# uibk-uncover/ws-unet

Hardware: AMD Instinct MI355X
Metric: 512x512 grayscale images/sec (UNet predict) (higher is better)
Workload: dtype f16 MFMA on the f16 halves + ONE block-scaled fp4 (e2m1) MFMA per tap pair for both residual cross terms (per-pixel / per-(co, tap) E8M0 scales), fp32 accumulate; planar storage

## Files before the change

ws_unet_amd/csrc/conv3x3_q.hip:

```cpp
#include "wsu_device.h"
#include <cstdlib>

namespace {

constexpr int TW = 32, TH = 16, IW = TW + 2, IH = TH + 2;
constexpr int NPIX = IW * IH;
constexpr int PLANE = NPIX * 16;
constexpr int IN_SEG = (NPIX + 63) / 64;
constexpr int S_LDS = IN_SEG * 256;
constexpr int IN_SLOT = 3 * PLANE + S_LDS;
constexpr int W_GRAN = 9 * 3 * WSU_COB * 16;
constexpr int W_SLOT = W_GRAN + 1024;
constexpr int NIN = 3, NWS = 2;
constexpr int W_BASE = NIN * IN_SLOT;
constexpr int LDS_EXTRA = W_BASE + NWS * W_SLOT;
constexpr int ZERO_BYTES = 3 * IW * 16 + 32;
constexpr int LDS_TOTAL = LDS_EXTRA + 1024 * 4 + 4 * 64 * 4 + 16 + ZERO_BYTES;
static_assert(LDS_TOTAL <= 160 * 1024 && W_SLOT % 1024 == 0, "LDS budget");
constexpr int NLOAD = 4;
constexpr int W_PIECES = W_SLOT / 1024;
constexpr unsigned OOB = 0xFFFFFFF0u;
constexpr int IN_SLOT_H = 2 * PLANE;
constexpr int W_SLOT_H = 9 * 2 * WSU_COB * 16;
template <int FMT> struct QGeo {
// ... 321 lines not shown
    auto q4_reads = [&](auto tp_c, auto ml_c, auto mu_c, u32x4* a4, u32x4* b4, int* sa, int* sb) __attribute__((always_inline)) {
        constexpr int tp = decltype(tp_c)::value, ML = decltype(ml_c)::value, MU = decltype(mu_c)::value;
        constexpr bool single = 2 * tp + 1 >= 9;
        constexpr int t0 = 2 * tp, pix0 = (t0 / 3) * IW + t0 % 3;
        constexpr unsigned wimm = (unsigned)((6 * tp + 2) * 64) * 16u;
        static_assert(!single || (wimm == W4_IMM && (unsigned)pix0 * 16u == B4_IMM), "tap 8");
        const unsigned wbase = single ? x_w4 : x_w, sabase = single ? x_sa4 : x_sa;
        const unsigned bbase = single ? x_b4 : (tp == 1 ? x_b2 : x_b1), sbbase = single ? x_sb0 : (tp == 1 ? x_sb2 : x_sb1);
_Pragma("unroll")
        for (int m = ML; m < MU; ++m) {
            a4[m] = *(lds_cu32x4*)(at(wbase) + wimm + m * 32 * 16);
            sa[m] = *(lds_cuchar*)(at(sabase) + 128 * tp + m * 32);
        }
_Pragma("unroll")
        for (int q = 0; q < RQ; ++q) {
            b4[q] = *(lds_cu32x4*)(at(bbase) + (pix0 + q * IW) * 16);
            sb[q] = *(lds_cint*)(at(sbbase) + (pix0 + q * IW) * 4);
        }
    };
    auto cross_q4 = [&](auto tp_c, auto ms_c, auto first_c) __attribute__((always_inline)) {
        constexpr int ms = decltype(ms_c)::value, ML = ms < 0 ? 0 : ms, MU = ms < 0 ? MH : ms + 1;
        constexpr bool FIRST = decltype(first_c)::value;
        u32x4 a4[2], b4[4]; int sa[2], sb[4];
        q4_reads(tp_c, std::integral_constant<int, ML>{}, std::integral_constant<int, MU>{}, a4, b4, sa, sb);
_Pragma("unroll")
        for (int m = ML; m < MU; ++m)
_Pragma("unroll")
            for (int q = 0; q < RQ; ++q) {
                if constexpr (FIRST) acc[m][q] = wsu_mfma_q4_z(a4[m], b4[q], sa[m], sb[q]);
                else wsu_mfma_q4(a4[m], b4[q], sa[m], sb[q], acc[m][q]);
            }
    };
    constexpr std::false_type not_first{};
    constexpr std::true_type tile_first{};
    auto units_range = [&](auto ms_c, auto lo_c, auto hi_c, auto first_c) __attribute__((always_inline)) {
        constexpr int lo = decltype(lo_c)::value, hi = decltype(hi_c)::value;
        constexpr bool FIRST = decltype(first_c)::value;
        static_assert(!FIRST || lo == 0, "a tile opens with tap pair 0");
        WSU_STATIC_FOR(hi - lo, i, {
            constexpr int tp = lo + i;
            if constexpr (!H) cross_q4(std::integral_constant<int, tp>{}, ms_c, std::integral_constant<bool, FIRST && tp == 0>{});
            main_term(std::integral_constant<int, 2 * tp>{}, ms_c, std::integral_constant<bool, FIRST && H && tp == 0>{});
            if constexpr (2 * tp + 1 < 9) main_term(std::integral_constant<int, 2 * tp + 1>{}, ms_c, not_first);
        });
    };
    constexpr std::integral_constant<int, -1> all_m{};
    struct Frag { u32x4 a[2]; u32x4 b[4]; int sa[2]; int sb[4]; };
    auto load_unit = [&](auto u_c, Frag& f, u32x4* row1) __attribute__((always_inline)) {
        constexpr int u = decltype(u_c)::value, tp = u / 3, k = u % 3;
        if constexpr (k == 0) {
            q4_reads(std::integral_constant<int, tp>{}, std::integral_constant<int, 0>{}, std::integral_constant<int, MH>{}, f.a, f.b, f.sa, f.sb);
        } else {
            constexpr int tap = 2 * tp + k - 1, dy = tap / 3, dx = tap % 3;
_Pragma("unroll")
            for (int m = 0; m < MH; ++m) f.a[m] = *(lds_cu32x4*)(at(a_off) + ((tap * 3) * 64 + m * 32) * 16);
            if constexpr (RQ == 2) {
                if constexpr (dy > 0) f.b[0] = row1[tap - 3];
                else f.b[0] = *(lds_cu32x4*)(at(b_off) + (dy * IW + dx) * 16);
                f.b[1] = row1[tap] = *(lds_cu32x4*)(at(b_off) + ((1 + dy) * IW + dx) * 16);
            } else {
_Pragma("unroll")
                for (int q = 0; q < RQ; ++q) f.b[q] = *(lds_cu32x4*)(at(b_off) + ((q + dy) * IW + dx) * 16);
            }
        }
    };
    auto mma_unit = [&](auto u_c, Frag& f, auto first_c) __attribute__((always_inline)) {
        constexpr int u = decltype(u_c)::value, k = u % 3;
        constexpr bool FIRST = decltype(first_c)::value && u == 0;
        if constexpr (k == 0) {
_Pragma("unroll")
            for (int m = 0; m < MH; ++m)
_Pragma("unroll")
                for (int q = 0; q < RQ; ++q) {
                    if constexpr (FIRST) acc[m][q] = wsu_mfma_q4_z(f.a[m], f.b[q], f.sa[m], f.sb[q]);
                    else wsu_mfma_q4(f.a[m], f.b[q], f.sa[m], f.sb[q], acc[m][q]);
                }
        } else {
_Pragma("unroll")
            for (int m = 0; m < MH; ++m)
_Pragma("unroll")
                for (int q = 0; q < RQ; ++q) wsu_mfma_f16(f.a[m], f.b[q], acc[m][q]);
        }
    };
    auto units_pipelined = [&](auto first_c) __attribute__((always_inline)) {
        constexpr int NU = 14;
        Frag fr[2];
        u32x4 row1[9];
        load_unit(std::integral_constant<int, 0>{}, fr[0], row1);
        WSU_STATIC_FOR(NU, u, {
            if constexpr (u + 1 < NU) load_unit(std::integral_constant<int, u + 1>{}, fr[(u + 1) % 2], row1);
            __builtin_amdgcn_sched_barrier(0);
            mma_unit(u_c, fr[u % 2], first_c);
            __builtin_amdgcn_sched_barrier(0);
        });
    };
    auto units_all = [&](auto ms_c, auto first_c) __attribute__((always_inline)) {
        if constexpr (PIPE && decltype(ms_c)::value < 0) { units_pipelined(first_c); return; }
        units_range(ms_c, std::integral_constant<int, 0>{}, std::integral_constant<int, 5>{}, first_c);
    };

    auto finish_tile = [&]() __attribute__((always_inline)) {
        int l31 = l31_k, hh = hh_k;
        asm volatile("" : "+v"(l31), "+v"(hh));
        const int col = cur.x0 + l31;
        const unsigned hw16 = (unsigned)(a.h * a.w) * 16u;
        const int nco = a.cout >> 4;
        float hz[4][HC > 0 ? HC : 1];
        float vmax = 0.f;
        const float relu_floor = a.relu ? 0.f : -__builtin_inff();
#pragma unroll
        for (int q = 0; q < RQ; ++q)
#pragma unroll
            for (int o = 0; o < (HC > 0 ? HC : 1); ++o) hz[q][o] = 0.f;
        struct QOff { unsigned g0, g1, q, s; };
        auto pair_off = [&](unsigned plane_bytes, unsigned off0, unsigned off1, unsigned soff0, unsigned soff1, bool ok0, bool ok1) __attribute__((always_inline)) {
            const unsigned hp = hh ? plane_bytes : 0u;
            const bool okm = hh ? ok1 : ok0;
            QOff o = {ok0 ? off0 + hp : OOB, ok1 ? off1 + hp : OOB, okm ? (hh ? off1 : off0) + 2u * plane_bytes : OOB, okm ? 3u * plane_bytes + (hh ? soff1 : soff0) : OOB};
            asm volatile("" : "+v"(o.g0), "+v"(o.g1), "+v"(o.q), "+v"(o.s));
            return o;
        };
        constexpr bool YQ = FQ && !H;
        QOff qo[RQ / 2] = {}, qop = {};
        if constexpr (YQ) {
            const unsigned sblk = (unsigned)(((cur.y0 >> 4) * a.tiles_x + (cur.x0 >> 5)) * 512);
_Pragma("unroll")
            for (int rp = 0; rp < RQ / 2; ++rp) {
                const int r0 = RQ * wv + 2 * rp, row0 = cur.y0 + r0;
                qo[rp] = pair_off(hw16, (unsigned)(row0 * a.w + col) * 16u, (unsigned)((row0 + 1) * a.w + col) * 16u,
                                  sblk + (unsigned)(r0 * 32 + l31), sblk + (unsigned)((r0 + 1) * 32 + l31), row0 < a.h && col < a.w, row0 + 1 < a.h && col < a.w);
            }
            if constexpr (POOL) {
                const int hp = a.h >> 1, wp2 = a.w >> 1, ptx = (wp2 + 31) >> 5;
                const int gy0 = (cur.y0 >> 1) + (RQ / 2) * wv, gx = (cur.x0 >> 1) + (l31 >> 1);
                const unsigned php16 = (unsigned)(hp * wp2) * 16u;
                if constexpr (RQ == 4) {
                    const bool okx = !(l31 & 1) && gx < wp2;
                    qop = pair_off(php16, (unsigned)(gy0 * wp2 + gx) * 16u, (unsigned)((gy0 + 1) * wp2 + gx) * 16u,
                                   wsu_q_soff(gy0, gx, ptx), wsu_q_soff(gy0 + 1, gx, ptx), okx && gy0 < hp, okx && gy0 + 1 < hp);
                } else {
                    const unsigned coff = (l31 & 1) ? (unsigned)wsu_q_chunk_bytes(hp, wp2) : 0u;
                    const unsigned off = (unsigned)(gy0 * wp2 + gx) * 16u + coff, soff = wsu_q_soff(gy0, gx, ptx) + coff;
                    const bool ok = gx < wp2 && gy0 < hp;
                    qop = {ok ? off + (hh ? php16 : 0u) : OOB, OOB, (ok && !hh) ? off + 2u * php16 : OOB, (ok && !hh) ? 3u * php16 + soff : OOB};
                    asm volatile("" : "+v"(qop.g0), "+v"(qop.q), "+v"(qop.s));
                }
            }
        }
        auto store_pair_q = [&](const f32x4& X0, const f32x4& Y0, const f32x4& X1, const f32x4& Y1, char* base, unsigned chunk_bytes, const QOff& o, bool have, bool fold) __attribute__((always_inline)) {
            u32x4 g0, g1; uint32_t dh0, dr0, sb0, dh1, dr1, sb1;
            const float mx0 = wsu_q4_pre(X0, Y0, g0, dh0, dr0, sb0);
            const float mx1 = wsu_q4_pre(X1, Y1, g1, dh1, dr1, sb1);
            if (fold) vmax = wsu_max3(vmax, mx0, mx1);
            const u32x4 qg = wsu_q4_pair(dh0, dr0, dh1, dr1);
            const auto rs = __builtin_amdgcn_make_buffer_rsrc(base, 0, have ? (int)chunk_bytes : 0, 0x00020000);
            __builtin_amdgcn_raw_buffer_store_b128(g0, rs, (int)o.g0, 0, 0);
            __builtin_amdgcn_raw_buffer_store_b128(g1, rs, (int)o.g1, 0, 0);
            __builtin_amdgcn_raw_buffer_store_b128(qg, rs, (int)o.q, 0, 0);
            __builtin_amdgcn_raw_buffer_store_b8((unsigned char)(hh ? sb1 : sb0), rs, (int)o.s, 0, 0);
        };
        auto store_one_q = [&](const f32x4& X, const f32x4& Y, char* base, unsigned chunk_bytes, const QOff& o) __attribute__((always_inline)) {
            u32x4 g; uint32_t dh, dr, sb;
            wsu_q4_pre(X, Y, g, dh, dr, sb);
            const u32x4 qg = wsu_q4_single(dh, dr);
            const auto rs = __builtin_amdgcn_make_buffer_rsrc(base, 0, (int)chunk_bytes, 0x00020000);
            __builtin_amdgcn_raw_buffer_store_b128(g, rs, (int)o.g0, 0, 0);
            __builtin_amdgcn_raw_buffer_store_b128(qg, rs, (int)o.q, 0, 0);
            __builtin_amdgcn_raw_buffer_store_b8((unsigned char)sb, rs, (int)o.s, 0, 0);
        };
        auto store_one_h = [&](const f32x4& X, const f32x4& Y, char* base, unsigned plane_bytes, unsigned off, bool ok, bool have) __attribute__((always_inline)) {
            const auto rs = __builtin_amdgcn_make_buffer_rsrc(base, 0, have ? (int)(2u * plane_bytes) : 0, 0x00020000);
            __builtin_amdgcn_raw_buffer_store_b128(wsu_h_granule(X, Y), rs, (int)(ok ? off + (hh ? plane_bytes : 0u) : OOB), 0, 0);
        };
        auto store_one_a = [&](const f32x4& X, const f32x4& Y, char* base, unsigned plane_bytes, unsigned off, bool ok, bool have) __attribute__((always_inline)) {
            uint32_t xh0, xh1, xlo, yh0, yh1, ylo;
            wsu_split4_f16r8(X, WSU_F8_XLO_DIV, xh0, xh1, xlo);
            wsu_split4_f16r8(Y, WSU_F8_XLO_DIV, yh0, yh1, ylo);
            wsu_swap32(xh0, yh0); wsu_swap32(xh1, yh1);
            uint32_t xlp = xlo, ylp = ylo;
            wsu_swap32(xlo, xlp); wsu_swap32(ylo, ylp);
// ... 59 lines not shown
                            const float cx = fmaxf(vx[0][e], vx[1][e]), cy = fmaxf(vy[0][e], vy[1][e]);
                            px[rp][e] = fmaxf(cx, dpp_xor1(cx)); py[rp][e] = fmaxf(cy, dpp_xor1(cy));
                        }
                    }
                });
                if constexpr (POOL) {
                    const int hp = a.h >> 1, wp2 = a.w >> 1;
                    const int gy0 = (cur.y0 >> 1) + (RQ / 2) * wv, gx = (cur.x0 >> 1) + (l31 >> 1);
                    const bool okx = !(l31 & 1) && gx < wp2;
                    const unsigned php16 = (unsigned)(hp * wp2) * 16u;
                    if constexpr (H) {
                        char* base = a.ypool + ((size_t)cur.n * nco + oc) * (2u * php16);
#pragma unroll
                        for (int rp = 0; rp < RQ / 2; ++rp)
                            store_one_h(px[rp], py[rp], base, php16, (unsigned)((gy0 + rp) * wp2 + gx) * 16u, okx && gy0 + rp < hp, true);
                    } else if constexpr (FQ) {
                        const unsigned cbp = (unsigned)wsu_q_chunk_bytes(hp, wp2);
                        char* base = a.ypool + ((size_t)cur.n * nco + oc) * cbp;
                        if constexpr (RQ == 4) {
                            store_pair_q(px[0], py[0], px[1], py[1], base, cbp, qop, true, false);
                        } else if constexpr (cp == 0) {
                            spx = px[0]; spy = py[0];
                        } else {
                            static_assert(cp == 1, "piece 1 closes the pair: its chunk follows piece 0's");
                            const bool odd = (l31 & 1) != 0;
                            f32x4 sx, sy;
_Pragma("unroll")
                            for (int e = 0; e < 4; ++e) { sx[e] = odd ? px[0][e] : spx[e]; sy[e] = odd ? py[0][e] : spy[e]; }
                            store_one_q(sx, sy, base - cbp, 2u * cbp, qop);
                        }
                    } else {
                        char* base = a.ypool + (((size_t)cur.n * nco + oc) * 3) * php16;
#pragma unroll
                        for (int rp = 0; rp < RQ / 2; ++rp)
                            store_one_a(px[rp], py[rp], base, php16, (unsigned)((gy0 + rp) * wp2 + gx) * 16u, okx && gy0 + rp < hp, true);
                    }
                }
            };
            piece(std::integral_constant<int, 0>{});
            piece(std::integral_constant<int, 1>{});
        };
        auto nothing = [](auto) __attribute__((always_inline)) {};
        if constexpr (EPO) {
            constexpr int NHT = 2 * (RQ / 2);
            epi_m(std::integral_constant<int, 0>{}, [&](auto h_c) __attribute__((always_inline)) {
                constexpr int h = decltype(h_c)::value;
                constexpr int lo = 5 * h / NHT, hi = 5 * (h + 1) / NHT;
                if constexpr (hi > lo) units_range(std::integral_constant<int, 1>{}, std::integral_constant<int, lo>{}, std::integral_constant<int, hi>{}, not_first);
            });
            epi_m(std::integral_constant<int, 1>{}, nothing);
        } else {
            WSU_STATIC_FOR(MH, m, { (void)m; epi_m(m_c, nothing); });
        }
        if constexpr (HEAD) {
            const size_t hw = (size_t)a.h * a.w;
#pragma unroll
            for (int q = 0; q < RQ; ++q) {
                const int row = cur.y0 + RQ * wv + q;
#pragma unroll
                for (int o = 0; o < HC; ++o)
                    if (HC == 1 || o < a.head_cout) {
                        uint32_t mine = __builtin_bit_cast(uint32_t, hz[q][o]), other = mine;
                        wsu_swap32(mine, other);
                        const float z = __builtin_bit_cast(float, mine) + __builtin_bit_cast(float, other) + s_hb[o];
                        if (!hh && row < a.h && col < a.w) {
                            const size_t plane = ((size_t)cur.n * a.head_cout + o) * hw;
                            const uint32_t off = (uint32_t)(row * a.w + col);
                            if (a.head_logit) (a.head_logit + plane)[off] = z;
                            (a.head_out + plane)[off] = 1.f / (1.f + expf(-z));
                        }
                    }
            }
        }
        if (a.range_flag && (a.y || POOL) && __builtin_amdgcn_ballot_w64(!(vmax <= (H ? WSU_F16_RANGE : WSU_F8_RANGE))) != 0 && lane == 0)
            atomicOr(a.range_flag, 1u);
        ++kt;
        if (j + 1 < J) cur = tile_of(a, lw + kt * G);
    };
    for (int t = 0; t < K; ++t) {
        if (a.nch == 1) {
            zero_acc();
        } else {
            begin_step(); units_all(all_m, tile_first); ++j;
            for (int cc = 2; cc < a.nch; ++cc) { begin_step(); units_all(all_m, not_first); ++j; }
        }
        begin_step();
        if constexpr (EPO) units_all(std::integral_constant<int, 0>{}, not_first);
        else units_all(all_m, not_first);
        __builtin_amdgcn_sched_barrier(0);
        finish_tile();
        ++j;
    }
}

__global__ void pack_conv3x3_f4_kernel(const float* __restrict__ w, char* __restrict__ dst, int cin, int cout) {
    const int nch = cin / 16;
    const long long total = (long long)(cout / WSU_COB) * nch * 9 * WSU_COB;
    for (long long d = (long long)blockIdx.x * blockDim.x + threadIdx.x; d < total; d += (long long)gridDim.x * blockDim.x) {
        long long t = d;
        const int co = (int)(t % WSU_COB); t /= WSU_COB;
        const int tap = (int)(t % 9); t /= 9;
        const int c = (int)(t % nch); const int cb = (int)(t / nch);
        float v[16], r[16];
        uint32_t h[8];
#pragma unroll
        for (int e = 0; e < 16; ++e) v[e] = w[(((size_t)(cb * WSU_COB + co) * cin + c * 16 + e) * 3 + tap / 3) * 3 + tap % 3];
#pragma unroll
        for (int e = 0; e < 8; ++e) {
            const _Float16 a = (_Float16)v[2 * e], b = (_Float16)v[2 * e + 1];
            h[e] = (uint32_t)__builtin_bit_cast(unsigned short, a) | ((uint32_t)__builtin_bit_cast(unsigned short, b) << 16);
            r[2 * e] = (v[2 * e] - (float)a) * 2048.f; r[2 * e + 1] = (v[2 * e + 1] - (float)b) * 2048.f;
        }
        const u32x4 h0 = mk_u4(h[0], h[1], h[2], h[3]), h1 = mk_u4(h[4], h[5], h[6], h[7]);
        const int E = wsu_q4_block_exp(wsu_f16x16_max_abs_bits(h0, h1));
        const float sc = wsu_pow2f(E);
        uint32_t q[4] = {0, 0, 0, 0};
        WSU_STATIC_FOR(8, e, { q[e >> 2] = __builtin_amdgcn_cvt_scalef32_pk_fp4_f32(q[e >> 2], r[2 * e], r[2 * e + 1], sc, e & 3); });
        q[2] = wsu_f16x8_to_fp4(h0, sc); q[3] = wsu_f16x8_to_fp4(h1, sc);
        char* slice = dst + ((size_t)cb * nch + c) * W_SLOT;
        char* base = slice + (size_t)(tap * 3) * (WSU_COB * 16) + co * 16;
        *reinterpret_cast<u32x4*>(base) = h0;
        *reinterpret_cast<u32x4*>(base + WSU_COB * 16) = h1;
        *reinterpret_cast<u32x4*>(base + 2 * WSU_COB * 16) = mk_u4(q[0], q[1], q[2], q[3]);
        slice[W_GRAN + tap * 64 + co] = (char)(E + 127 - 11);
        if (tap == 0 && co < 7) *reinterpret_cast<u32x4*>(slice + W_GRAN + 576 + co * 64) = mk_u4(0, 0, 0, 0), *reinterpret_cast<u32x4*>(slice + W_GRAN + 576 + co * 64 + 16) = mk_u4(0, 0, 0, 0),
            *reinterpret_cast<u32x4*>(slice + W_GRAN + 576 + co * 64 + 32) = mk_u4(0, 0, 0, 0), *reinterpret_cast<u32x4*>(slice + W_GRAN + 576 + co * 64 + 48) = mk_u4(0, 0, 0, 0);
    }
}

__global__ void pack_conv3x3_h_kernel(const float* __restrict__ w, char* __restrict__ dst, int cin, int cout) {
    const int nch = cin / 16;
    const long long total = (long long)(cout / WSU_COB) * nch * 9 * WSU_COB;
    for (long long d = (long long)blockIdx.x * blockDim.x + threadIdx.x; d < total; d += (long long)gridDim.x * blockDim.x) {
        long long t = d;
        const int co = (int)(t % WSU_COB); t /= WSU_COB;
        const int tap = (int)(t % 9); t /= 9;
        const int c = (int)(t % nch); const int cb = (int)(t / nch);
        uint32_t h[8];
#pragma unroll
        for (int e = 0; e < 8; ++e) {
            const size_t i0 = (((size_t)(cb * WSU_COB + co) * cin + c * 16 + 2 * e) * 3 + tap / 3) * 3 + tap % 3;
            const _Float16 a = (_Float16)w[i0], b = (_Float16)w[i0 + 9];
            h[e] = (uint32_t)__builtin_bit_cast(unsigned short, a) | ((uint32_t)__builtin_bit_cast(unsigned short, b) << 16);
        }
        char* base = dst + ((size_t)cb * nch + c) * W_SLOT_H + (size_t)(tap * 2) * (WSU_COB * 16) + co * 16;
        *reinterpret_cast<u32x4*>(base) = mk_u4(h[0], h[1], h[2], h[3]);
        *reinterpret_cast<u32x4*>(base + WSU_COB * 16) = mk_u4(h[4], h[5], h[6], h[7]);
    }
}

#define WSU_Q_VARIANTS_RQ(X, RQ)                    \
    X(RQ, 0, false, false, false, false, WSU_PLANAR_Q) \
    X(RQ, 0, false, true, false, false, WSU_PLANAR_Q)  \
    X(RQ, 0, true, false, false, false, WSU_PLANAR_Q)  \
    X(RQ, 0, true, true, false, false, WSU_PLANAR_Q)   \
    X(RQ, 1, false, false, false, false, WSU_PLANAR_Q) \
    X(RQ, 4, false, false, false, false, WSU_PLANAR_Q) \
    X(RQ, 0, false, false, true, false, WSU_PLANAR_Q)  \
    X(RQ, 0, false, true, true, false, WSU_PLANAR_Q)
#define WSU_Q_VARIANTS(X)                            \
    WSU_Q_VARIANTS_RQ(X, 4)                          \
    WSU_Q_VARIANTS_RQ(X, 2)                          \
    X(2, 0, true, true, false, true, WSU_PLANAR_Q)   \
    X(2, 0, false, true, false, false, WSU_PLANAR_H) \
    X(2, 0, true, true, false, false, WSU_PLANAR_H)  \
    X(2, 1, false, true, false, false, WSU_PLANAR_H) \
    X(2, 4, false, true, false, false, WSU_PLANAR_H) \
// ... 135 lines not shown
```

ws_unet_amd/csrc/conv3x3_qu.hip:

```cpp
#include "wsu_device.h"

namespace {

constexpr int TW = 32, TH = 16;
constexpr int CW = 17, CH = 9, CPIX = CW * CH;
constexpr int NPIX_S = 4 * CPIX;
constexpr int PLANE_S = NPIX_S * 16;
constexpr int SEG_S = (NPIX_S + 63) / 64;
constexpr int IN_S = 3 * PLANE_S + SEG_S * 256;
constexpr int LP = 33, LH = TH / 2 + 2, LW_ = TW / 2 + 2;
constexpr int NPIX_L = LP * LH;
constexpr int PLANE_L = NPIX_L * 16;
constexpr int SEG_L = (NPIX_L + 63) / 64;
constexpr int IN_L = 3 * PLANE_L + SEG_L * 256;
constexpr int W_GRAN_S = 9 * 3 * WSU_COB * 16;
constexpr int W_S = W_GRAN_S + 1024;
constexpr int W_UNITS_L = 8;
constexpr int W_GRAN_L = W_UNITS_L * 3 * WSU_COB * 16;
constexpr int W_L = W_GRAN_L + 1024;
constexpr int PIECES_S = W_S / 1024, PIECES_L = W_L / 1024;
constexpr int REGION = 80640;
constexpr int OFF_SW = IN_S, OFF_LIN = W_L, OFF_LW1 = W_L + IN_L;
constexpr int LDS_BIAS = 2 * REGION;
constexpr int MAX_COUT = 512;
// ... 221 lines not shown
    };
    unsigned a_off = 0, b_off = 0, hd_w = 0, hd_sa = 0, hd_b = 0, hd_sb = 0, x_w = 0, x_w4 = 0, x_sa = 0, x_sa4 = 0, x_b4 = 0;
    constexpr unsigned W4_IMM = (unsigned)((8 * 3 + 2) * 64) * 16u;
    unsigned tap_sel[5] = {};
    if constexpr (!H) {
        WSU_STATIC_FOR(5, tp, {
            constexpr int t0 = 2 * tp, t1 = (2 * tp + 1 < 9) ? 2 * tp + 1 : 2 * tp;
            tap_sel[tp] = ((hh ? tap_s(t1 / 3, t1 % 3) : tap_s(t0 / 3, t0 % 3)) + laneS) >> 2;
            asm volatile("" : "+v"(tap_sel[tp]));
        });
    }
    auto sync_step = [&](auto low_c) __attribute__((always_inline)) {
        constexpr bool LOW = decltype(low_c)::value;
        const unsigned r = next_region();
        in_off = LOW ? r + OFF_LIN : r;
        w_off = LOW ? r : r + OFF_SW;
        hh_q = hh;
        asm volatile("" : "+v"(hh_q));
        a_off = Lb + w_off + (unsigned)l31 * 16u + (unsigned)hh * 1024u;
        b_off = Lb + in_off + (unsigned)hh * (LOW ? PLANE_L : PLANE_S) + (LOW ? laneL : laneS);
        if constexpr (!H && !LOW) {
            const unsigned hq = (unsigned)hh_q, zero = Lb + (unsigned)LDS_ZERO;
            const unsigned w0 = Lb + w_off + (unsigned)l31 * 16u;
            x_w = w0 + hq * (unsigned)(3 * 64 * 16);
            x_w4 = hq ? zero - W4_IMM : w0;
            x_sa4 = Lb + w_off + W_GRAN_S + (unsigned)l31;
            x_sa = x_sa4 + hq * 64u;
            hd_b = Lb + in_off + 2 * PLANE_S + tap_sel[0] * 4u;
            hd_sb = Lb + in_off + 3 * PLANE_S + tap_sel[0];
            x_b4 = hq ? zero : Lb + in_off + 2 * PLANE_S + tap_sel[4] * 4u;
            asm volatile("" : "+v"(a_off), "+v"(b_off), "+v"(x_w), "+v"(x_w4), "+v"(x_sa), "+v"(x_sa4), "+v"(hd_b), "+v"(hd_sb), "+v"(x_b4));
        } else if constexpr (!H) {
            const int u = cls * 2 + hh_q;
            const unsigned pb = (unsigned)((py * LP + px) * 16) + (unsigned)hh_q * 16u + laneL;
            hd_w = Lb + w_off + (unsigned)((u * 3 + 2) * 64 + l31) * 16u;
            hd_sa = Lb + w_off + W_GRAN_L + (unsigned)(u * 64 + l31);
            hd_b = Lb + in_off + 2 * PLANE_L + pb;
            hd_sb = Lb + in_off + 3 * PLANE_L + (pb >> 2);
            asm volatile("" : "+v"(a_off), "+v"(b_off), "+v"(hd_w), "+v"(hd_sa), "+v"(hd_b), "+v"(hd_sb));
        } else {
            asm volatile("" : "+v"(a_off), "+v"(b_off));
        }
        __builtin_amdgcn_s_barrier();
        asm volatile("" ::: "memory");
    };
    struct Frag { u32x4 a[2]; u32x4 b[2]; int sa[2]; int sb[2]; };
    auto load_unit = [&](auto u_c, Frag& f) __attribute__((always_inline)) {
        constexpr int u = decltype(u_c)::value, tp = u / 3, k = u % 3;
        if constexpr (k == 0) {
            constexpr bool single = 2 * tp + 1 >= 9;
            constexpr unsigned wimm = (unsigned)((6 * tp + 2) * 64) * 16u;
            static_assert(!single || wimm == W4_IMM, "tap 8");
            const unsigned wb = single ? x_w4 : x_w, sab = single ? x_sa4 : x_sa;
            const unsigned bb = tp == 0 ? hd_b : (single ? x_b4 : Lb + in_off + 2 * PLANE_S + tap_sel[tp] * 4u);
            const unsigned sbb = tp == 0 ? hd_sb : Lb + in_off + 3 * PLANE_S + tap_sel[tp];
_Pragma("unroll")
            for (int m = 0; m < 2; ++m) { f.a[m] = *(lds_cu32x4*)(at(wb) + wimm + m * 512); f.sa[m] = *(lds_cuchar*)(at(sab) + 128 * tp + m * 32); }
_Pragma("unroll")
            for (int q = 0; q < 2; ++q) {
                f.b[q] = *(lds_cu32x4*)(at(bb) + q * QS);
                f.sb[q] = *(lds_cint*)(at(sbb) + q * (QS >> 2));
            }
        } else {
            constexpr int tap = 2 * tp + k - 1;
            const unsigned pb = b_off + tap_s(tap / 3, tap % 3);
_Pragma("unroll")
            for (int m = 0; m < 2; ++m) f.a[m] = *(lds_cu32x4*)(at(a_off) + ((tap * WPL) * 64) * 16 + m * 512);
_Pragma("unroll")
            for (int q = 0; q < 2; ++q) f.b[q] = *(lds_cu32x4*)(at(pb) + q * QS);
        }
    };
    auto mma_unit = [&](auto u_c, Frag& f, auto first_c) __attribute__((always_inline)) {
        constexpr int u = decltype(u_c)::value, k = u % 3;
        constexpr bool FIRST = decltype(first_c)::value && u == 0;
_Pragma("unroll")
        for (int m = 0; m < 2; ++m)
_Pragma("unroll")
            for (int q = 0; q < 2; ++q) {
                if constexpr (k != 0) wsu_mfma_f16(f.a[m], f.b[q], acc[m][q]);
                else if constexpr (FIRST) acc[m][q] = wsu_mfma_q4_z(f.a[m], f.b[q], f.sa[m], f.sb[q]);
                else wsu_mfma_q4(f.a[m], f.b[q], f.sa[m], f.sb[q], acc[m][q]);
            }
    };
    auto skip_units = [&](auto first_c) __attribute__((always_inline)) {
        constexpr bool FIRST = decltype(first_c)::value;
        if constexpr (!H) {
            constexpr int NU = 14;
            Frag fr[2];
            load_unit(std::integral_constant<int, 0>{}, fr[0]);
            WSU_STATIC_FOR(NU, u, {
                if constexpr (u + 1 < NU) load_unit(std::integral_constant<int, u + 1>{}, fr[(u + 1) % 2]);
                __builtin_amdgcn_sched_barrier(0);
                mma_unit(u_c, fr[u % 2], first_c);
                __builtin_amdgcn_sched_barrier(0);
            });
        } else {
            WSU_STATIC_FOR(9, tap, {
                u32x4 ah[2], bh[2];
                const unsigned pb = b_off + tap_s(tap / 3, tap % 3);
_Pragma("unroll")
                for (int m = 0; m < 2; ++m) ah[m] = *(lds_cu32x4*)(at(a_off) + ((tap * WPL) * 64) * 16 + m * 512);
_Pragma("unroll")
                for (int q = 0; q < 2; ++q) bh[q] = *(lds_cu32x4*)(at(pb) + q * QS);
_Pragma("unroll")
                for (int m = 0; m < 2; ++m)
_Pragma("unroll")
                    for (int q = 0; q < 2; ++q) {
                        if constexpr (FIRST && tap == 0) acc[m][q] = wsu_mfma_f16_z(ah[m], bh[q]);
                        else wsu_mfma_f16(ah[m], bh[q], acc[m][q]);
                    }
            });
        }
    };
    auto low_units = [&](auto dy_c) __attribute__((always_inline)) {
        constexpr int dy = decltype(dy_c)::value;
        constexpr unsigned WDY = dy ? (unsigned)(OFF_LW1) : 0u;
        const unsigned rowo = (unsigned)(((py + dy) * LP + px) * 16);
        if constexpr (!H) {
            const int u = cls * 2 + hh_q;
            u32x4 a4[2], b4[2]; int sa[2], sb[2];
            const unsigned pb = rowo + (unsigned)hh_q * 16u + laneL;
            const unsigned wb = dy == 0 ? hd_w : Lb + w_off + WDY + (unsigned)((u * 3 + 2) * 64 + l31) * 16u;
            const unsigned sab = dy == 0 ? hd_sa : Lb + w_off + WDY + W_GRAN_L + (unsigned)(u * 64 + l31);
            const unsigned bb = dy == 0 ? hd_b : Lb + in_off + 2 * PLANE_L + pb;
            const unsigned sbb = dy == 0 ? hd_sb : Lb + in_off + 3 * PLANE_L + (pb >> 2);
_Pragma("unroll")
            for (int m = 0; m < 2; ++m) { a4[m] = *(lds_cu32x4*)(at(wb) + m * 512); sa[m] = *(lds_cuchar*)(at(sab) + m * 32); }
_Pragma("unroll")
            for (int q = 0; q < 2; ++q) {
                b4[q] = *(lds_cu32x4*)(at(bb) + q * QL);
                sb[q] = *(lds_cint*)(at(sbb) + q * (QL >> 2));
            }
_Pragma("unroll")
            for (int m = 0; m < 2; ++m)
_Pragma("unroll")
                for (int q = 0; q < 2; ++q) wsu_mfma_q4(a4[m], b4[q], sa[m], sb[q], acc[m][q]);
        }
        WSU_STATIC_FOR(2, dx, {
            u32x4 ah[2], bh[2];
            const unsigned wb = a_off + WDY + (unsigned)(((cls * 2 + dx) * WPL) * 64) * 16u;
            const unsigned pb = b_off + rowo + dx * 16u;
_Pragma("unroll")
            for (int m = 0; m < 2; ++m) ah[m] = *(lds_cu32x4*)(at(wb) + m * 512);
_Pragma("unroll")
            for (int q = 0; q < 2; ++q) bh[q] = *(lds_cu32x4*)(at(pb) + q * QL);
_Pragma("unroll")
            for (int m = 0; m < 2; ++m)
_Pragma("unroll")
                for (int q = 0; q < 2; ++q) wsu_mfma_f16(ah[m], bh[q], acc[m][q]);
        });
    };

    auto finish_tile = [&]() __attribute__((always_inline)) {
        int l31o = l31, hho = hh, lro = lrow, lco = lcol;
        asm volatile("" : "+v"(l31o), "+v"(hho), "+v"(lro), "+v"(lco));
        const unsigned hw16 = (unsigned)(a.h * a.w) * 16u;
        const unsigned cbytes = (unsigned)wsu_q_chunk_bytes(a.h, a.w);
        const int nco = a.cout >> 4;
        const int X = cur.x0 + 2 * lco + px;
        const int Y0 = cur.y0 + 2 * (4 * rh + lro) + py, Y1 = Y0 + 4;
        const bool ok0 = Y0 < a.h && X < a.w, ok1 = Y1 < a.h && X < a.w;
        const unsigned off0 = (unsigned)(Y0 * a.w + X) * 16u, off1 = (unsigned)(Y1 * a.w + X) * 16u;
        const unsigned so0 = wsu_q_soff(Y0, X, a.tiles_x), so1 = wsu_q_soff(Y1, X, a.tiles_x);
        const unsigned hpl = hho ? hw16 : 0u;
        const bool okm = hho ? ok1 : ok0;
        unsigned og0 = ok0 ? off0 + hpl : OOB, og1 = ok1 ? off1 + hpl : OOB;
        unsigned oq = okm ? (hho ? off1 : off0) + 2u * hw16 : OOB, os = okm ? 3u * hw16 + (hho ? so1 : so0) : OOB;
        asm volatile("" : "+v"(og0), "+v"(og1), "+v"(oq), "+v"(os));
        const float relu_floor = a.relu ? 0.f : -__builtin_inff();
        float vmax = 0.f;
        WSU_STATIC_FOR(2, m, {
            WSU_STATIC_FOR(2, cp, {
                const int oc = cur.cb * 4 + m * 2 + cp;
                const int co0 = oc * 16 + 4 * hho;
                const f32x4 bx = *reinterpret_cast<const f32x4*>(s_bias + co0), by = *reinterpret_cast<const f32x4*>(s_bias + co0 + 8);
                f32x4 vx[2], vy[2];
_Pragma("unroll")
                for (int q = 0; q < 2; ++q)
_Pragma("unroll")
                    for (int e = 0; e < 4; ++e) {
                        const float x = fmaxf(acc[m][q][8 * cp + e] + bx[e], relu_floor), y = fmaxf(acc[m][q][8 * cp + 4 + e] + by[e], relu_floor);
                        vx[q][e] = x; vy[q][e] = y;
                        if constexpr (H) vmax = fmaxf(fmaxf(vmax, fabsf(x)), fabsf(y));
                    }
                if constexpr (H) {
                    char* base = a.y + ((size_t)cur.n * nco + oc) * (2u * hw16);
                    const auto rs = __builtin_amdgcn_make_buffer_rsrc(base, 0, (int)(2u * hw16), 0x00020000);
                    __builtin_amdgcn_raw_buffer_store_b128(wsu_h_granule(vx[0], vy[0]), rs, (int)og0, 0, 0);
                    __builtin_amdgcn_raw_buffer_store_b128(wsu_h_granule(vx[1], vy[1]), rs, (int)og1, 0, 0);
                    return;
                }
                u32x4 g0, g1; uint32_t dh0, dr0, sb0, dh1, dr1, sb1;
                const float mx0 = wsu_q4_pre(vx[0], vy[0], g0, dh0, dr0, sb0);
                const float mx1 = wsu_q4_pre(vx[1], vy[1], g1, dh1, dr1, sb1);
                vmax = wsu_max3(vmax, mx0, mx1);
                const u32x4 qg = wsu_q4_pair(dh0, dr0, dh1, dr1);
                char* base = a.y + ((size_t)cur.n * nco + oc) * cbytes;
                const auto rs = __builtin_amdgcn_make_buffer_rsrc(base, 0, (int)cbytes, 0x00020000);
                __builtin_amdgcn_raw_buffer_store_b128(g0, rs, (int)og0, 0, 0);
                __builtin_amdgcn_raw_buffer_store_b128(g1, rs, (int)og1, 0, 0);
                __builtin_amdgcn_raw_buffer_store_b128(qg, rs, (int)oq, 0, 0);
                __builtin_amdgcn_raw_buffer_store_b8((unsigned char)(hho ? sb1 : sb0), rs, (int)os, 0, 0);
            });
        });
        if (a.range_flag && __builtin_amdgcn_ballot_w64(!(vmax <= (H ? WSU_F16_RANGE : WSU_F8_RANGE))) != 0 && lane == 0) atomicOr(a.range_flag, 1u);
    };

    for (int t = 0; t < K; ++t) {
        sync_step(std::false_type{});
        skip_units(std::true_type{});
        for (int c = 1; c < a.nchS; ++c) {
            sync_step(std::false_type{});
            skip_units(std::false_type{});
        }
        for (int c = 0; c < a.nchL; ++c) {
            sync_step(std::true_type{});
            low_units(std::integral_constant<int, 0>{});
            low_units(std::integral_constant<int, 1>{});
        }
        finish_tile();
        if (t + 1 < K) cur = tile_of(a, lw + (t + 1) * G);
    }
}

template <int FMT>
__global__ void pack_up_low_kernel(const float* __restrict__ w3, const float* __restrict__ wt, char* __restrict__ dst, float* __restrict__ wc_dense,
                                   int cup, int c2, int cl, int cout) {
    const int nchL = cl / 16, ctot = cup + c2;
    const long long total = (long long)(cout / WSU_COB) * nchL * 2 * W_UNITS_L * WSU_COB;
    for (long long d = (long long)blockIdx.x * blockDim.x + threadIdx.x; d < total; d += (long long)gridDim.x * blockDim.x) {
        long long t = d;
        const int co = (int)(t % WSU_COB); t /= WSU_COB;
        const int u = (int)(t % W_UNITS_L); t /= W_UNITS_L;
        const int dy = (int)(t & 1); t >>= 1;
        const int c = (int)(t % nchL); const int cb = (int)(t / nchL);
        const int cls = u >> 1, dx = u & 1, py = cls >> 1, px = cls & 1;
        const int ky0 = py == 0 ? (dy == 0 ? 0 : 1) : (dy == 0 ? 0 : 2), ky1 = py == 0 ? (dy == 0 ? 0 : 2) : (dy == 0 ? 1 : 2);
        const int kx0 = px == 0 ? (dx == 0 ? 0 : 1) : (dx == 0 ? 0 : 2), kx1 = px == 0 ? (dx == 0 ? 0 : 2) : (dx == 0 ? 1 : 2);
        const int cog = cb * WSU_COB + co;
        float v[16], r[16];
#pragma unroll
        for (int e = 0; e < 16; ++e) v[e] = 0.f;
        for (int ci = 0; ci < cup; ++ci)
            for (int ky = ky0; ky <= ky1; ++ky)
                for (int kx = kx0; kx <= kx1; ++kx) {
                    const float w = w3[(((size_t)cog * ctot + ci) * 3 + ky) * 3 + kx];
                    const int sy = (py + ky + 1) & 1, sx = (px + kx + 1) & 1;
#pragma unroll
                    for (int e = 0; e < 16; ++e) v[e] = fmaf(w, wt[(((size_t)(c * 16 + e) * cup + ci) * 2 + sy) * 2 + sx], v[e]);
                }
        if (wc_dense)
#pragma unroll
            for (int e = 0; e < 16; ++e) wc_dense[((((size_t)cog * cl + c * 16 + e) * 2 + py) * 2 + px) * 4 + dy * 2 + dx] = v[e];
        uint32_t h[8];
#pragma unroll
        for (int e = 0; e < 8; ++e) {
            const _Float16 x = (_Float16)v[2 * e], y = (_Float16)v[2 * e + 1];
            h[e] = (uint32_t)__builtin_bit_cast(unsigned short, x) | ((uint32_t)__builtin_bit_cast(unsigned short, y) << 16);
            r[2 * e] = (v[2 * e] - (float)x) * 2048.f; r[2 * e + 1] = (v[2 * e + 1] - (float)y) * 2048.f;
        }
        const u32x4 h0 = mk_u4(h[0], h[1], h[2], h[3]), h1 = mk_u4(h[4], h[5], h[6], h[7]);
        if constexpr (FMT == WSU_PLANAR_H) {
            char* base = dst + (((size_t)cb * nchL + c) * 2 + dy) * W_L_H + (size_t)(u * 2) * (WSU_COB * 16) + co * 16;
            *reinterpret_cast<u32x4*>(base) = h0;
            *reinterpret_cast<u32x4*>(base + WSU_COB * 16) = h1;
            continue;
        }
        const int E = wsu_q4_block_exp(wsu_f16x16_max_abs_bits(h0, h1));
        const float sc = wsu_pow2f(E);
        uint32_t q[4] = {0, 0, 0, 0};
        WSU_STATIC_FOR(8, e, { q[e >> 2] = __builtin_amdgcn_cvt_scalef32_pk_fp4_f32(q[e >> 2], r[2 * e], r[2 * e + 1], sc, e & 3); });
        q[2] = wsu_f16x8_to_fp4(h0, sc); q[3] = wsu_f16x8_to_fp4(h1, sc);
        char* slice = dst + (((size_t)cb * nchL + c) * 2 + dy) * W_L;
        char* base = slice + (size_t)(u * 3) * (WSU_COB * 16) + co * 16;
        *reinterpret_cast<u32x4*>(base) = h0;
        *reinterpret_cast<u32x4*>(base + WSU_COB * 16) = h1;
        *reinterpret_cast<u32x4*>(base + 2 * WSU_COB * 16) = mk_u4(q[0], q[1], q[2], q[3]);
        slice[W_GRAN_L + u * 64 + co] = (char)(E + 127 - 11);
        if (u == 0 && co < 32) *reinterpret_cast<u32x4*>(slice + W_GRAN_L + 512 + co * 16) = mk_u4(0, 0, 0, 0);
    }
}

__global__ void up_bias_kernel(const float* __restrict__ w3, const float* __restrict__ bt, const float* __restrict__ b3, float* __restrict__ out, int cup, int c2, int cout) {
    const int co = blockIdx.x * blockDim.x + threadIdx.x;
    if (co >= cout) return;
    float s = b3 ? b3[co] : 0.f;
    if (bt)
        for (int ci = 0; ci < cup; ++ci) {
            float t = 0.f;
            for (int k = 0; k < 9; ++k) t += w3[((size_t)co * (cup + c2) + ci) * 9 + k];
            s = fmaf(bt[ci], t, s);
        }
    out[co] = s;
}

struct UFormat {
// ... 93 lines not shown
```

Measured before the change: 3819.

## Carry last f16 MMA unit across channel-chunk sync into next step

In the pipelined conv3x3 Q kernels, the final MMA unit of a channel chunk is deferred: its fragments are kept in registers and issued after the next chunk's first load, so those MFMAs overlap the barrier and LDS load latency of the next step. A trailing carried MMA flushes the last deferred unit. This costs extra VGPRs for the carried fragments and adds more control paths. Ordering changes in the qu kernel for the last skip chunk and the nchS==1 path need care.

```diff
diff --git a/ws_unet_amd/csrc/conv3x3_q.hip b/ws_unet_amd/csrc/conv3x3_q.hip
--- a/ws_unet_amd/csrc/conv3x3_q.hip
+++ b/ws_unet_amd/csrc/conv3x3_q.hip
@@ -427,20 +427,46 @@
                 for (int q = 0; q < RQ; ++q) wsu_mfma_f16(f.a[m], f.b[q], acc[m][q]);
         }
     };
-    auto units_pipelined = [&](auto first_c) __attribute__((always_inline)) {
+    constexpr bool CARRY = PIPE && RQ == 2;
+    u32x4 ca[2], cb[2];
+    auto carried_mma = [&]() __attribute__((always_inline)) {
+_Pragma("unroll")
+        for (int m = 0; m < MH; ++m)
+_Pragma("unroll")
+            for (int q = 0; q < 2; ++q) wsu_mfma_f16(ca[m], cb[q], acc[m][q]);
+    };
+    auto units_pipelined = [&](auto first_c, auto cin_c, auto cout_c) __attribute__((always_inline)) {
         constexpr int NU = 14;
+        constexpr bool CIN = decltype(cin_c)::value, COUT = decltype(cout_c)::value;
+        static_assert(!(CIN || COUT) || CARRY, "the carried unit: RQ = 2, format Q");
         Frag fr[2];
         u32x4 row1[9];
         load_unit(std::integral_constant<int, 0>{}, fr[0], row1);
+        if constexpr (CIN) {
+            __builtin_amdgcn_sched_barrier(0);
+            carried_mma();
+            __builtin_amdgcn_sched_barrier(0);
+        }
         WSU_STATIC_FOR(NU, u, {
             if constexpr (u + 1 < NU) load_unit(std::integral_constant<int, u + 1>{}, fr[(u + 1) % 2], row1);
             __builtin_amdgcn_sched_barrier(0);
-            mma_unit(u_c, fr[u % 2], first_c);
+            if constexpr (!(COUT && u == NU - 1)) mma_unit(u_c, fr[u % 2], first_c);
             __builtin_amdgcn_sched_barrier(0);
         });
-    };
+        if constexpr (COUT) {
+            ca[0] = fr[(NU - 1) % 2].a[0]; cb[0] = fr[(NU - 1) % 2].b[0]; cb[1] = fr[(NU - 1) % 2].b[1];
+            if constexpr (MH == 2) {
+                ca[1] = fr[(NU - 1) % 2].a[1];
+                asm volatile("s_waitcnt lgkmcnt(0)" : "+v"(ca[0]), "+v"(ca[1]), "+v"(cb[0]), "+v"(cb[1]) :: "memory");
+            } else {
+                asm volatile("s_waitcnt lgkmcnt(0)" : "+v"(ca[0]), "+v"(cb[0]), "+v"(cb[1]) :: "memory");
+            }
+        }
+    };
+    constexpr std::false_type no_carry{};
+    constexpr std::true_type carry{};
     auto units_all = [&](auto ms_c, auto first_c) __attribute__((always_inline)) {
-        if constexpr (PIPE && decltype(ms_c)::value < 0) { units_pipelined(first_c); return; }
+        if constexpr (PIPE && decltype(ms_c)::value < 0) { units_pipelined(first_c, no_carry, no_carry); return; }
         units_range(ms_c, std::integral_constant<int, 0>{}, std::integral_constant<int, 5>{}, first_c);
     };
 
@@ -666,7 +692,19 @@
             zero_acc();
         } else {
             begin_step(); units_all(all_m, tile_first); ++j;
-            for (int cc = 2; cc < a.nch; ++cc) { begin_step(); units_all(all_m, not_first); ++j; }
+            if constexpr (CARRY) {
+                if (a.nch > 2) {
+                    if constexpr (MH == 2) asm volatile("" : "=v"(ca[0]), "=v"(ca[1]), "=v"(cb[0]), "=v"(cb[1]));
+                    else asm volatile("" : "=v"(ca[0]), "=v"(cb[0]), "=v"(cb[1]));
+                    begin_step(); units_pipelined(not_first, no_carry, carry); ++j;
+                    for (int cc = 3; cc < a.nch; ++cc) { begin_step(); units_pipelined(not_first, carry, carry); ++j; }
+                    __builtin_amdgcn_sched_barrier(0);
+                    carried_mma();
+                    __builtin_amdgcn_sched_barrier(0);
+                }
+            } else {
+                for (int cc = 2; cc < a.nch; ++cc) { begin_step(); units_all(all_m, not_first); ++j; }
+            }
         }
         begin_step();
         if constexpr (EPO) units_all(std::integral_constant<int, 0>{}, not_first);
diff --git a/ws_unet_amd/csrc/conv3x3_qu.hip b/ws_unet_amd/csrc/conv3x3_qu.hip
--- a/ws_unet_amd/csrc/conv3x3_qu.hip
+++ b/ws_unet_amd/csrc/conv3x3_qu.hip
@@ -327,18 +327,37 @@
                 else wsu_mfma_q4(f.a[m], f.b[q], f.sa[m], f.sb[q], acc[m][q]);
             }
     };
-    auto skip_units = [&](auto first_c) __attribute__((always_inline)) {
+    constexpr bool CARRY = !H;
+    u32x4 ca[2], cb[2];
+    auto carried_mma = [&]() __attribute__((always_inline)) {
+_Pragma("unroll")
+        for (int m = 0; m < 2; ++m)
+_Pragma("unroll")
+            for (int q = 0; q < 2; ++q) wsu_mfma_f16(ca[m], cb[q], acc[m][q]);
+    };
+    auto skip_units = [&](auto first_c, auto cin_c, auto cout_c) __attribute__((always_inline)) {
         constexpr bool FIRST = decltype(first_c)::value;
+        constexpr bool CIN = decltype(cin_c)::value, COUT = decltype(cout_c)::value;
+        static_assert(!(CIN || COUT) || CARRY, "the carried unit: format Q");
         if constexpr (!H) {
             constexpr int NU = 14;
             Frag fr[2];
             load_unit(std::integral_constant<int, 0>{}, fr[0]);
+            if constexpr (CIN) {
+                __builtin_amdgcn_sched_barrier(0);
+                carried_mma();
+                __builtin_amdgcn_sched_barrier(0);
+            }
             WSU_STATIC_FOR(NU, u, {
                 if constexpr (u + 1 < NU) load_unit(std::integral_constant<int, u + 1>{}, fr[(u + 1) % 2]);
                 __builtin_amdgcn_sched_barrier(0);
-                mma_unit(u_c, fr[u % 2], first_c);
+                if constexpr (!(COUT && u == NU - 1)) mma_unit(u_c, fr[u % 2], first_c);
                 __builtin_amdgcn_sched_barrier(0);
             });
+            if constexpr (COUT) {
+                ca[0] = fr[(NU - 1) % 2].a[0]; ca[1] = fr[(NU - 1) % 2].a[1]; cb[0] = fr[(NU - 1) % 2].b[0]; cb[1] = fr[(NU - 1) % 2].b[1];
+                asm volatile("s_waitcnt lgkmcnt(0)" : "+v"(ca[0]), "+v"(ca[1]), "+v"(cb[0]), "+v"(cb[1]) :: "memory");
+            }
         } else {
             WSU_STATIC_FOR(9, tap, {
                 u32x4 ah[2], bh[2];
@@ -452,11 +471,28 @@
     };
 
     for (int t = 0; t < K; ++t) {
-        sync_step(std::false_type{});
-        skip_units(std::true_type{});
-        for (int c = 1; c < a.nchS; ++c) {
+        if constexpr (CARRY) {
+            asm volatile("" : "=v"(ca[0]), "=v"(ca[1]), "=v"(cb[0]), "=v"(cb[1]));
             sync_step(std::false_type{});
-            skip_units(std::false_type{});
+            skip_units(std::true_type{}, std::false_type{}, std::true_type{});
+            for (int c = 2; c < a.nchS; ++c) {
+                sync_step(std::false_type{});
+                skip_units(std::false_type{}, std::true_type{}, std::true_type{});
+            }
+            __builtin_amdgcn_sched_barrier(0);
+            carried_mma();
+            __builtin_amdgcn_sched_barrier(0);
+            if (a.nchS > 1) {
+                sync_step(std::false_type{});
+                skip_units(std::false_type{}, std::false_type{}, std::false_type{});
+            }
+        } else {
+            sync_step(std::false_type{});
+            skip_units(std::true_type{}, std::false_type{}, std::false_type{});
+            for (int c = 1; c < a.nchS; ++c) {
+                sync_step(std::false_type{});
+                skip_units(std::false_type{}, std::false_type{}, std::false_type{});
+            }
         }
         for (int c = 0; c < a.nchL; ++c) {
             sync_step(std::true_type{});
```

Result: no change. 3823, median of 6 (+0.1%).
